# moberweger/deep-prior-pp

Measured on AMD Instinct MI355X. Metric: depth-crops/sec (NYU ResNet50 bs128) 1/2/4/8 GPU; mean 3D joint err (mm), higher is better.
Workload: dtype f32; 1 GPU; NYU posereg_embedding ResNet (type 0, 30-D PCA prior) train step: fused augment + fwd + bwd + ADAM, bs128/GPU fp32, 128x128x1 crops; global_batch=128, parallelism=dp1, augment=True, augment_pipelined=True, bn=local per-GPU batch statistics, launch_mode=native

## Files before the change

deep-prior-pp_amd/csrc/gemm_expand.hip:

```cpp
#include "gemm_args.h"

namespace {

template <int KT, bool BKC, bool IT2, bool ACT, bool RES, bool BNB, bool LZ = false, bool PB = false, bool ST = false>
__global__ __launch_bounds__(DPP_THREADS) DPP_WAVES_PER_EU(1, 2) void gemm_expand_kernel(GemmArgs ga, int rpw) {
    static_assert(!PB || ((KT % 32 == 0 || KT == 16) && !LZ), "bf16 MFMA operands: whole 32-deep steps, or K = 16 with a zero upper half");
    dpp_kernarg_warm<sizeof(GemmArgs)>();
    const dpp_gemm_desc& d = ga.d;
    constexpr int KL = KT / 4, KV = KL / 4;
    constexpr int RT = 2, RI = 16 * RT;
    const int lane = threadIdx.x & 63, l15 = lane & 15, kq = lane >> 4;
    const int NG = d.N >> 6, nblk = d.M / rpw;
    const int gw = blockIdx.x * 4 + (threadIdx.x >> 6);
    if (gw >= NG * nblk) return;
    const int cg = gw % NG, rblk = gw / NG;
    const int n0 = cg * 64 + 4 * l15;
    const int wrow0 = rblk * rpw, iters = rpw / RI;
    const dpp_epilogue& ep = d.epi;
    const int modeA = ACT ? d.actA.mode : 0;
    const bool relu_mask = BNB && ep.bn_relu != 0;
    const bool a16 = ST && !LZ && ga.shA != 0, c16 = ST && (d.store & DPP_ST_C) != 0, x16 = ST && (d.store & DPP_ST_BNX) != 0;
    dpp_stamp(ga.prof, 0);

    float bw[4][KL];
    if (BKC) {
#pragma unroll
        for (int ct = 0; ct < 4; ++ct)
#pragma unroll
            for (int j = 0; j < KV; ++j) {
                const float4 t = *reinterpret_cast<const float4*>(d.B + (size_t)(n0 + ct) * d.ldb + kq * KL + 4 * j);
                bw[ct][4 * j] = t.x; bw[ct][4 * j + 1] = t.y; bw[ct][4 * j + 2] = t.z; bw[ct][4 * j + 3] = t.w;
            }
    } else {
#pragma unroll
        for (int e = 0; e < KL; ++e) {
            const float4 t = *reinterpret_cast<const float4*>(d.B + (size_t)(kq * KL + e) * d.ldb + n0);
            bw[0][e] = t.x; bw[1][e] = t.y; bw[2][e] = t.z; bw[3][e] = t.w;
        }
    }
    constexpr int KS = PB ? (KL + 7) / 8 : 1;
    dpp_bf16x8 bwp[4][KS];
    if (PB) {
#pragma unroll
        for (int ct = 0; ct < 4; ++ct)
#pragma unroll
            for (int ss = 0; ss < KS; ++ss)
#pragma unroll
                for (int q = 0; q < 8; ++q) bwp[ct][ss][q] = (dpp_bf16)(ss * 8 + q < KL ? bw[ct][ss * 8 + q < KL ? ss * 8 + q : 0] : 0.0f);
    }
    struct Regs { float4 a[RT][KV]; float4 a2[RT][LZ ? KV : 1]; float4 res[RT][4]; float4 bx[RT][4]; };
    auto fetch = [&](Regs& g, int it) {
        const int r0 = wrow0 + it * RI;
#pragma unroll
        for (int rt = 0; rt < RT; ++rt) {
            const size_t oa = (size_t)(r0 + rt * 16 + l15) * d.lda + kq * KL;
            if (a16) {
#pragma unroll
                for (int j = 0; j < KV; ++j) g.a[rt][j] = dpp_raw8(d.A + ((oa + 4 * j) >> 1));
            } else {
#pragma unroll
                for (int j = 0; j < KV; ++j) {
                    g.a[rt][j] = *reinterpret_cast<const float4*>(d.A + oa + 4 * j);
                    if (LZ) g.a2[rt][j] = *reinterpret_cast<const float4*>(d.actA.x2 + oa + 4 * j);
                }
            }
        }
#pragma unroll
        for (int rt = 0; rt < RT; ++rt)
#pragma unroll
            for (int r = 0; r < 4; ++r) {
                const size_t o = (size_t)(r0 + rt * 16 + kq * 4 + r) * d.ldc + n0;
                if (RES) g.res[rt][r] = c16 ? dpp_raw8(d.residual + (o >> 1)) : *reinterpret_cast<const float4*>(d.residual + o);
                if (BNB) g.bx[rt][r] = x16 ? dpp_raw8(ep.bn_x + (o >> 1)) : *reinterpret_cast<const float4*>(ep.bn_x + o);
            }
    };
    Regs g0, g1;
    fetch(g0, 0);
    float4 mu[KV], sc[KV], be[KV], ax[LZ ? KV : 1];
#pragma unroll
    for (int j = 0; j < KV; ++j) {
        mu[j] = sc[j] = be[j] = make_float4(0.f, 0.f, 0.f, 0.f);
        if (LZ || (modeA & 2)) {
            mu[j] = *reinterpret_cast<const float4*>(d.actA.mean + kq * KL + 4 * j);
            sc[j] = *reinterpret_cast<const float4*>(d.actA.scale + kq * KL + 4 * j);
            be[j] = *reinterpret_cast<const float4*>(d.actA.beta + kq * KL + 4 * j);
        }
        if (LZ) ax[j] = *reinterpret_cast<const float4*>(d.actA.aux + kq * KL + 4 * j);
    }
    const bool lz_store = LZ && d.actA.out != nullptr && cg == 0;
    float4 cbias = make_float4(0.f, 0.f, 0.f, 0.f), cmean = cbias, cscale = cbias, cbeta = cbias, cistd = cbias;
    if (d.bias) cbias = *reinterpret_cast<const float4*>(d.bias + n0);
    if (BNB) {
        cmean = *reinterpret_cast<const float4*>(ep.bn_mean + n0); cscale = *reinterpret_cast<const float4*>(ep.bn_scale + n0);
        cbeta = *reinterpret_cast<const float4*>(ep.bn_beta + n0); cistd = *reinterpret_cast<const float4*>(ep.bn_inv_std + n0);
    }
    dpp_stamp(ga.prof, 1);

    float sx[4] = {0.f, 0.f, 0.f, 0.f}, sy[4] = {0.f, 0.f, 0.f, 0.f};
    float rmean[4] = {0.f, 0.f, 0.f, 0.f}, rm2[4] = {0.f, 0.f, 0.f, 0.f};
    const bool want_stats = ep.stats != nullptr;
    auto colsum = [&](float (&s)[4]) {
#pragma unroll
        for (int j = 0; j < 4; ++j) { s[j] += __shfl_xor(s[j], 16); s[j] += __shfl_xor(s[j], 32); }
    };

    auto step = [&](Regs& g, int it) {
        const int r0 = wrow0 + it * RI;
        f32x4 acc[RT][4];
#pragma unroll
        for (int rt = 0; rt < RT; ++rt)
#pragma unroll
            for (int ct = 0; ct < 4; ++ct) acc[rt][ct] = (f32x4){0.f, 0.f, 0.f, 0.f};
        dpp_bf16x8 ap[RT][KS];
        if (PB && KL < 8) {
#pragma unroll
            for (int rt = 0; rt < RT; ++rt)
#pragma unroll
                for (int q = 0; q < 8; ++q) ap[rt][0][q] = (dpp_bf16)0.0f;
        }
#pragma unroll
        for (int j = 0; j < KV; ++j) {
            float av[RT][4];
#pragma unroll
            for (int rt = 0; rt < RT; ++rt) {
                float4 v = a16 ? dpp_widen4(g.a[rt][j]) : g.a[rt][j];
                if (LZ) {
                    const float4 x = g.a2[rt][j];
                    v = make_float4(sc[j].x * v.x - ax[j].x * (x.x - mu[j].x) - be[j].x, sc[j].y * v.y - ax[j].y * (x.y - mu[j].y) - be[j].y,
                                    sc[j].z * v.z - ax[j].z * (x.z - mu[j].z) - be[j].z, sc[j].w * v.w - ax[j].w * (x.w - mu[j].w) - be[j].w);
                    if (lz_store) *reinterpret_cast<float4*>(d.actA.out + (size_t)(r0 + rt * 16 + l15) * d.lda + kq * KL + 4 * j) = v;
                }
                if (modeA & 2) {
                    v.x = dpp_fma(v.x - mu[j].x, sc[j].x, be[j].x); v.y = dpp_fma(v.y - mu[j].y, sc[j].y, be[j].y);
                    v.z = dpp_fma(v.z - mu[j].z, sc[j].z, be[j].z); v.w = dpp_fma(v.w - mu[j].w, sc[j].w, be[j].w);
                }
                if (modeA & 1) { v.x = fmaxf(v.x, 0.f); v.y = fmaxf(v.y, 0.f); v.z = fmaxf(v.z, 0.f); v.w = fmaxf(v.w, 0.f); }
                av[rt][0] = v.x; av[rt][1] = v.y; av[rt][2] = v.z; av[rt][3] = v.w;
                if (PB) {
#pragma unroll
                    for (int t = 0; t < 4; ++t) ap[rt][j / 2][(j & 1) * 4 + t] = (dpp_bf16)av[rt][t];
                }
            }
            if (PB) {
                if ((j & 1) || KL < 8) {
#pragma unroll
                    for (int rt = 0; rt < RT; ++rt)
#pragma unroll
                        for (int ct = 0; ct < 4; ++ct)
                            acc[rt][ct] = __builtin_amdgcn_mfma_f32_16x16x32_bf16(ap[rt][j / 2], bwp[ct][j / 2], acc[rt][ct], 0, 0, 0);
                }
            } else {
#pragma unroll
                for (int t = 0; t < 4; ++t)
#pragma unroll
                    for (int rt = 0; rt < RT; ++rt)
#pragma unroll
                        for (int ct = 0; ct < 4; ++ct)
                            acc[rt][ct] = __builtin_amdgcn_mfma_f32_16x16x4f32(av[rt][t], bw[ct][4 * j + t], acc[rt][ct], 0, 0, 0);
            }
        }
        float vals[RT][4][4];
#pragma unroll
        for (int rt = 0; rt < RT; ++rt)
#pragma unroll
            for (int r = 0; r < 4; ++r) {
                float v[4] = {acc[rt][0][r] + cbias.x, acc[rt][1][r] + cbias.y, acc[rt][2][r] + cbias.z, acc[rt][3][r] + cbias.w};
                if (RES) {
                    const float4 rr = c16 ? dpp_widen4(g.res[rt][r]) : g.res[rt][r];
                    v[0] += rr.x; v[1] += rr.y; v[2] += rr.z; v[3] += rr.w;
                }
                if (BNB) {
                    const float4 bxv = x16 ? dpp_widen4(g.bx[rt][r]) : g.bx[rt][r];
                    const float x[4] = {bxv.x, bxv.y, bxv.z, bxv.w};
                    const float cm[4] = {cmean.x, cmean.y, cmean.z, cmean.w}, cs[4] = {cscale.x, cscale.y, cscale.z, cscale.w};
                    const float cb[4] = {cbeta.x, cbeta.y, cbeta.z, cbeta.w}, ci[4] = {cistd.x, cistd.y, cistd.z, cistd.w};
#pragma unroll
                    for (int j = 0; j < 4; ++j) {
                        const float dx = x[j] - cm[j];
                        if (relu_mask && dx * cs[j] + cb[j] < 0.0f) v[j] = 0.0f;
                        if (c16) v[j] = dpp_bf16_round(v[j]);
                        sx[j] += v[j];
                        sy[j] += v[j] * (dx * ci[j]);
                    }
                }
                {
                    const size_t oc = (size_t)(r0 + rt * 16 + kq * 4 + r) * d.ldc + n0;
                    if (c16) dpp_st4(reinterpret_cast<dpp_bf16*>(d.C) + oc, make_float4(v[0], v[1], v[2], v[3]));
                    else *reinterpret_cast<float4*>(d.C + oc) = make_float4(v[0], v[1], v[2], v[3]);
                }
#pragma unroll
                for (int j = 0; j < 4; ++j) vals[rt][r][j] = v[j];
            }
        if (want_stats) {
            float sm[4] = {0.f, 0.f, 0.f, 0.f}, m2[4] = {0.f, 0.f, 0.f, 0.f};
#pragma unroll
            for (int rt = 0; rt < RT; ++rt)
#pragma unroll
                for (int r = 0; r < 4; ++r)
#pragma unroll
                    for (int j = 0; j < 4; ++j) sm[j] += vals[rt][r][j];
            colsum(sm);
#pragma unroll
            for (int j = 0; j < 4; ++j) sm[j] *= 1.0f / (float)RI;
#pragma unroll
            for (int rt = 0; rt < RT; ++rt)
#pragma unroll
                for (int r = 0; r < 4; ++r)
#pragma unroll
                    for (int j = 0; j < 4; ++j) { const float dv = vals[rt][r][j] - sm[j]; m2[j] += dv * dv; }
            colsum(m2);
            if (it == 0) {
#pragma unroll
                for (int j = 0; j < 4; ++j) { rmean[j] = sm[j]; rm2[j] = m2[j]; }
            } else {
                const float na = (float)(it * RI), nb = (float)RI, nn = na + nb;
#pragma unroll
                for (int j = 0; j < 4; ++j) {
                    const float dl = sm[j] - rmean[j];
                    rmean[j] += dl * (nb / nn);
                    rm2[j] += m2[j] + dl * dl * (na * nb / nn);
                }
            }
        }
    };

    if (IT2) {
        for (int it = 0; it < iters; it += 2) {
            if (it + 1 < iters) fetch(g1, it + 1);
            DPP_SCHED_FENCE();
            step(g0, it);
            if (it + 1 < iters) {
                if (it + 2 < iters) fetch(g0, it + 2);
                DPP_SCHED_FENCE();
                step(g1, it + 1);
            }
        }
    } else {
        DPP_SCHED_FENCE();
        step(g0, 0);
    }
    dpp_stamp(ga.prof, 3);
    if (BNB && ep.bn_partial != nullptr) {
        float tx[4] = {sx[0], sx[1], sx[2], sx[3]}, ty[4] = {sy[0], sy[1], sy[2], sy[3]};
        colsum(tx);
        colsum(ty);
        if (kq == 0) {
#pragma unroll
            for (int j = 0; j < 4; ++j) {
                ep.bn_partial[dpp_partial_index(0, n0 + j, rblk, d.N, nblk)] = tx[j];
                ep.bn_partial[dpp_partial_index(1, n0 + j, rblk, d.N, nblk)] = ty[j];
            }
        }
    }
    if (want_stats && kq == 0) {
#pragma unroll
        for (int j = 0; j < 4; ++j) {
            ep.stats[dpp_partial_index(0, n0 + j, rblk, d.N, nblk)] = rmean[j];
            ep.stats[dpp_partial_index(1, n0 + j, rblk, d.N, nblk)] = rm2[j];
        }
    }
    dpp_stamp(ga.prof, 4);
}

}

int dpp_gemm_expand_rows(const dpp_gemm_desc& d, const GemmArgs& ga) {
    if ((d.store & DPP_ST_B) || (d.store && (d.actA.mode & 4))) return 0;
    if (!d.a_kc || d.splitk != 1 || !d.C || !ga.vecA || !ga.vecB || !ga.wide) return 0;
    if (d.K != 16 && d.K != 32 && d.K != 64) return 0;
    if (d.N % 64 || d.M % 32) return 0;
    if (d.mapA.s != 1 || d.mapB.s != 1 || d.mapC.s != 1 || d.actB.mode != 0) return 0;
    if (d.actA.mode != 0 && d.actA.cmod < d.K) return 0;
    if (d.epi.stats && d.epi.bn_x) return 0;
    if (d.b_kc ? (d.epi.bn_x != nullptr || (d.actA.mode & 4)) : (d.actA.mode != 0 && d.actA.mode != 4)) return 0;
    if (d.actA.mode == 4 && d.actA.out && d.lda != d.K) return 0;
    if (d.precision != 0 && (d.precision != 1 || (d.actA.mode & 4))) return 0;
    int rpw = d.bm;
    if (rpw <= 0) rpw = d.M >= 65536 ? 128 : (d.M >= 16384 ? 64 : 32);
    if (rpw % 32 || d.M % rpw) return 0;
    return rpw;
}

namespace {

template <int KT>
int launch_expand(const GemmArgs& ga, int rpw, hipStream_t st) {
    const dpp_gemm_desc& d = ga.d;
    const int waves = (d.M / rpw) * (d.N / 64);
    const dim3 grid(dpp_cdiv(waves, 4));
    const bool it2 = rpw > 32, act = d.actA.mode != 0, res = d.residual != nullptr, bnb = d.epi.bn_x != nullptr, lz = d.actA.mode == 4;
    const bool pb = d.precision == 1;
    const bool stg = d.store != 0;
#define DPP_EXS(K_, I_, A_, R_, B_, L_, P_, S_) DPP_LAUNCH((gemm_expand_kernel<KT, K_, I_, A_, R_, B_, L_, P_, S_>), grid, dim3(DPP_THREADS), 0, st, ga, rpw)
#define DPP_EX(K_, I_, A_, R_, B_, L_, P_) do { if (!(L_) && stg) DPP_EXS(K_, I_, A_, R_, B_, L_, P_, !(L_)); else DPP_EXS(K_, I_, A_, R_, B_, L_, P_, false); } while (0)
#define DPP_EX_P(K_, I_, A_, R_, B_) do { if (pb) { DPP_EX(K_, I_, A_, R_, B_, false, true); break; } \
                                          DPP_EX(K_, I_, A_, R_, B_, false, false); } while (0)
#define DPP_EX_I(K_, A_, R_, B_, L_) do { if (L_) { if (it2) DPP_EX(K_, true, A_, R_, B_, true, false); else DPP_EX(K_, false, A_, R_, B_, true, false); } \
                                          else if (it2) DPP_EX_P(K_, true, A_, R_, B_); else DPP_EX_P(K_, false, A_, R_, B_); } while (0)
#define DPP_EX_R(K_, A_, B_, L_) do { if (res) DPP_EX_I(K_, A_, true, B_, L_); else DPP_EX_I(K_, A_, false, B_, L_); } while (0)
    if (d.b_kc) {
        if (act) DPP_EX_R(true, true, false, false); else DPP_EX_R(true, false, false, false);
    } else if (lz) {
        if (bnb) DPP_EX_R(false, false, true, true); else DPP_EX_R(false, false, false, true);
    } else {
        if (bnb) DPP_EX_R(false, false, true, false); else DPP_EX_R(false, false, false, false);
    }
#undef DPP_EX_P
#undef DPP_EXS
#undef DPP_EX_R
#undef DPP_EX_I
#undef DPP_EX
    return dpp_launch_status();
}

}

int dpp_gemm_expand_launch(const GemmArgs& ga, int rpw, hipStream_t st) {
    const dpp_gemm_desc& d = ga.d;
    return d.K == 64 ? launch_expand<64>(ga, rpw, st) : (d.K == 32 ? launch_expand<32>(ga, rpw, st) : launch_expand<16>(ga, rpw, st));
}
```

deep-prior-pp_amd/csrc/stem.hip:

```cpp
#include "dpp_common.h"

namespace {

constexpr int KS = 5, PAD = 2, NTAP = 25, KPAD = 28;
constexpr int TC = 16;
constexpr int LX = TC + 2 * PAD;
constexpr int LXP = LX + 1;

template <int CN>
__global__ __launch_bounds__(DPP_THREADS) void stem_fwd_kernel(const float* __restrict__ X, int N, int H, int W, const float* __restrict__ Wk,
                                                               const float* __restrict__ bias, int Co, float* __restrict__ Y,
                                                               uint8_t* __restrict__ arg, int tiles_x, int tiles_y,
                                                               float* __restrict__ stats, int y16) {
    dpp_kernarg_warm<128>();
    __shared__ float xs[LX * LXP];
    __shared__ float Ws[KPAD * CN * 16];
    const int tid = threadIdx.x, wave = tid >> 6, lane = tid & 63, l15 = lane & 15, kq = lane >> 4;
    const int bx = blockIdx.x % tiles_x, by = (blockIdx.x / tiles_x) % tiles_y, n = blockIdx.x / (tiles_x * tiles_y);
    const int cy0 = by * TC, cx0 = bx * TC;
    const int Hp = H >> 1, Wp = W >> 1;
    const float* img = X + (size_t)n * H * W;
    for (int s = tid; s < LX * LX; s += DPP_THREADS) {
        int hy = s / LX, hx = s - hy * LX;
        int y = cy0 + hy - PAD, x = cx0 + hx - PAD;
        xs[hy * LXP + hx] = (y >= 0 && y < H && x >= 0 && x < W) ? img[(size_t)y * W + x] : 0.0f;
    }
    for (int s = tid; s < KPAD * CN * 16; s += DPP_THREADS) {
        int k = s / (CN * 16), o = s - k * (CN * 16);
        Ws[s] = (k < NTAP && o < Co) ? Wk[(size_t)o * NTAP + k] : 0.0f;
    }
    __syncthreads();

    float bf[7][CN];
#pragma unroll
    for (int t = 0; t < 7; ++t)
#pragma unroll
        for (int ct = 0; ct < CN; ++ct) bf[t][ct] = Ws[(4 * t + kq) * (CN * 16) + ct * 16 + l15];
    int koff[7];
    bool kval[7];
#pragma unroll
    for (int t = 0; t < 7; ++t) {
        int k = 4 * t + kq;
        kval[t] = k < NTAP;
        int kk = kval[t] ? k : 0;
        koff[t] = (kk / KS) * LXP + (kk % KS);
    }

    float vals[4][CN];
#pragma unroll
    for (int i = 0; i < 4; ++i)
#pragma unroll
        for (int j = 0; j < CN; ++j) vals[i][j] = 0.0f;
#pragma unroll
    for (int rt = 0; rt < 4; ++rt) {
        const int ply = 2 * wave + (rt >> 1);
        const int qa = l15 >> 2, pa = l15 & 3;
        const int ay = 2 * ply + (pa >> 1), ax = 2 * (((rt & 1) << 2) + qa) + (pa & 1);
        const int abase = ay * LXP + ax;
        f32x4 acc[CN];
#pragma unroll
        for (int ct = 0; ct < CN; ++ct) acc[ct] = (f32x4){0.f, 0.f, 0.f, 0.f};
#pragma unroll
        for (int t = 0; t < 7; ++t) {
            float av = kval[t] ? xs[abase + koff[t]] : 0.0f;
#pragma unroll
            for (int ct = 0; ct < CN; ++ct) acc[ct] = __builtin_amdgcn_mfma_f32_16x16x4f32(av, bf[t][ct], acc[ct], 0, 0, 0);
        }
        const int py = (cy0 >> 1) + ply, px = (cx0 >> 1) + ((rt & 1) << 2) + kq;
        if (py < Hp && px < Wp) {
            size_t o = (((size_t)n * Hp + py) * Wp + px) * Co;
#pragma unroll
            for (int ct = 0; ct < CN; ++ct) {
                int col = ct * 16 + l15;
                if (col < Co) {
                    float best = fmaxf(fmaxf(acc[ct][0], acc[ct][1]), fmaxf(acc[ct][2], acc[ct][3]));
                    int ties = 0;
#pragma unroll
                    for (int r = 0; r < 4; ++r) ties |= (acc[ct][r] == best) ? (1 << r) : 0;
                    if (y16) reinterpret_cast<dpp_bf16*>(Y)[o + col] = (dpp_bf16)(best + bias[col]);
                    else Y[o + col] = best + bias[col];
                    vals[rt][ct] = best + bias[col];
                    if (arg) arg[o + col] = (uint8_t)ties;
                }
            }
        }
    }
    if (stats != nullptr) {
        float sm[CN], m2[CN];
#pragma unroll
        for (int ct = 0; ct < CN; ++ct) sm[ct] = vals[0][ct] + vals[1][ct] + vals[2][ct] + vals[3][ct];
        dpp_tile_colsum<CN, 4, 1, CN * 16>(sm, xs, wave, 0, l15, kq);
#pragma unroll
        for (int ct = 0; ct < CN; ++ct) {
            sm[ct] *= (1.0f / 64.0f);
            float t = 0.0f;
#pragma unroll
            for (int rt = 0; rt < 4; ++rt) { float dv = vals[rt][ct] - sm[ct]; t += dv * dv; }
            m2[ct] = t;
        }
        dpp_tile_colsum<CN, 4, 1, CN * 16>(m2, xs, wave, 0, l15, kq);
        if (kq == 0 && wave == 0) {
#pragma unroll
            for (int ct = 0; ct < CN; ++ct) {
                int col = ct * 16 + l15;
                if (col < Co) {
                    stats[dpp_partial_index(0, col, blockIdx.x, Co, gridDim.x)] = sm[ct];
                    stats[dpp_partial_index(1, col, blockIdx.x, Co, gridDim.x)] = m2[ct];
                }
            }
        }
    }
}

constexpr int LXW = LX + 2;
constexpr int GM_A = 64 * 32 + 16;

__global__ __launch_bounds__(DPP_THREADS) void stem_wgrad_kernel(const float* __restrict__ X, int N, int H, int W, const float* __restrict__ dY,
                                                                 const uint8_t* __restrict__ arg, int Co, float* __restrict__ partial,
                                                                 int tiles_x, int tiles_y, int tiles_per_block, int total_tiles) {
    dpp_kernarg_warm<128>();
    __shared__ __attribute__((aligned(16))) float gm[4 * GM_A];
    __shared__ float xs[LX * LXW];
    const int tid = threadIdx.x, wave = tid >> 6, lane = tid & 63, l15 = lane & 15, kq = lane >> 4;
    const int Hp = H >> 1, Wp = W >> 1;
    const bool vec = (Co & 3) == 0 && (reinterpret_cast<uintptr_t>(dY) & 15) == 0 && (reinterpret_cast<uintptr_t>(arg) & 3) == 0;
    int offB[2];
    bool okB[2];
#pragma unroll
    for (int ct = 0; ct < 2; ++ct) {
        const int tap = ct * 16 + l15;
        okB[ct] = tap < NTAP;
        const int tt = okB[ct] ? tap : 0;
        offB[ct] = ((kq >> 1) + tt / KS) * LXW + (kq & 1) + tt % KS;
    }
    float4 rg[2];
    unsigned rt_[2];
    float rh[2];
    auto load_tile = [&](int tile) {
        const int bx = tile % tiles_x, by = (tile / tiles_x) % tiles_y, n = tile / (tiles_x * tiles_y);
        const int cy0 = by * TC, cx0 = bx * TC;
#pragma unroll
        for (int i = 0; i < 2; ++i) {
            const int item = tid + i * DPP_THREADS, p = item >> 3, oq = item & 7;
            const int py = (cy0 >> 1) + (p >> 3), px = (cx0 >> 1) + (p & 7);
            float4 g = make_float4(0.f, 0.f, 0.f, 0.f);
            unsigned t = 0;
            if (py < Hp && px < Wp && oq * 4 < Co) {
                const size_t idx = (((size_t)n * Hp + py) * Wp + px) * Co + oq * 4;
                if (vec) {
                    g = *reinterpret_cast<const float4*>(dY + idx);
                    t = *reinterpret_cast<const unsigned*>(arg + idx);
                } else {
                    float gv[4] = {0.f, 0.f, 0.f, 0.f};
                    for (int j = 0; j < 4; ++j)
                        if (oq * 4 + j < Co) { gv[j] = dY[idx + j]; t |= (unsigned)arg[idx + j] << (8 * j); }
                    g = make_float4(gv[0], gv[1], gv[2], gv[3]);
                }
            }
            rg[i] = g;
            rt_[i] = t;
        }
        const float* img = X + (size_t)n * H * W;
#pragma unroll
        for (int i = 0; i < 2; ++i) {
            const int s2 = tid + i * DPP_THREADS;
            float v = 0.0f;
            if (s2 < LX * LX) {
                const int hy = s2 / LX, hx = s2 - hy * LX;
                const int y = cy0 + hy - PAD, x = cx0 + hx - PAD;
                if (y >= 0 && y < H && x >= 0 && x < W) v = img[(size_t)y * W + x];
            }
            rh[i] = v;
        }
    };
    auto commit_tile = [&]() {
#pragma unroll
        for (int i = 0; i < 2; ++i) {
            const int item = tid + i * DPP_THREADS, p = item >> 3, oq = item & 7;
            const float4 g = rg[i];
            const unsigned t = rt_[i];
#pragma unroll
            for (int a = 0; a < 4; ++a) {
                float4 m;
                m.x = ((t >> a) & 1u) ? g.x : 0.0f;
                m.y = ((t >> (8 + a)) & 1u) ? g.y : 0.0f;
                m.z = ((t >> (16 + a)) & 1u) ? g.z : 0.0f;
                m.w = ((t >> (24 + a)) & 1u) ? g.w : 0.0f;
                *reinterpret_cast<float4*>(&gm[a * GM_A + p * 32 + oq * 4]) = m;
            }
        }
#pragma unroll
        for (int i = 0; i < 2; ++i) {
            const int s2 = tid + i * DPP_THREADS;
            if (s2 < LX * LX) xs[(s2 / LX) * LXW + s2 % LX] = rh[i];
        }
    };
    f32x4 acc[2][2];
#pragma unroll
    for (int i = 0; i < 2; ++i)
#pragma unroll
        for (int j = 0; j < 2; ++j) acc[i][j] = (f32x4){0.f, 0.f, 0.f, 0.f};
    const int tile0 = blockIdx.x * tiles_per_block;
    int ntiles = total_tiles - tile0;
    if (ntiles > tiles_per_block) ntiles = tiles_per_block;
    if (ntiles > 0) load_tile(tile0);
    for (int ti = 0; ti < ntiles; ++ti) {
        commit_tile();
        __syncthreads();
        if (ti + 1 < ntiles) load_tile(tile0 + ti + 1);
#pragma unroll
        for (int sidx = 0; sidx < 16; ++sidx) {
            const int p = wave * 16 + sidx;
            const int base = (2 * (p >> 3)) * LXW + 2 * (p & 7);
            const float a0 = gm[kq * GM_A + p * 32 + l15], a1 = gm[kq * GM_A + p * 32 + 16 + l15];
            const float b0 = okB[0] ? xs[base + offB[0]] : 0.0f;
            const float b1 = okB[1] ? xs[base + offB[1]] : 0.0f;
            acc[0][0] = __builtin_amdgcn_mfma_f32_16x16x4f32(a0, b0, acc[0][0], 0, 0, 0);
            acc[0][1] = __builtin_amdgcn_mfma_f32_16x16x4f32(a0, b1, acc[0][1], 0, 0, 0);
            acc[1][0] = __builtin_amdgcn_mfma_f32_16x16x4f32(a1, b0, acc[1][0], 0, 0, 0);
            acc[1][1] = __builtin_amdgcn_mfma_f32_16x16x4f32(a1, b1, acc[1][1], 0, 0, 0);
        }
        __syncthreads();
    }
    float* red = gm;
#pragma unroll
    for (int rt = 0; rt < 2; ++rt)
#pragma unroll
        for (int ct = 0; ct < 2; ++ct)
#pragma unroll
            for (int r = 0; r < 4; ++r) red[wave * 1024 + (rt * 16 + kq * 4 + r) * 32 + ct * 16 + l15] = acc[rt][ct][r];
    __syncthreads();
    for (int s2 = tid; s2 < Co * NTAP; s2 += DPP_THREADS) {
        const int oo = s2 / NTAP, k = s2 - oo * NTAP;
        const int at = oo * 32 + k;
        partial[(size_t)blockIdx.x * Co * NTAP + s2] = ((red[at] + red[1024 + at]) + red[2048 + at]) + red[3072 + at];
    }
}

}

extern "C" int dpp_stem_fwd(const float* X, int N, int H, int W, const float* Wk, const float* bias, int Co, float* Y, uint8_t* argmax,
                            float* stats, int store,
                            dpp_stream_t stream) {
    if (!X || !Wk || !bias || !Y || N < 1 || H < 2 || W < 2 || (H & 1) || (W & 1) || Co < 1 || Co > 32 || (store & ~DPP_ST_C)) return DPP_E_BADARG;
    const int y16 = (store & DPP_ST_C) ? 1 : 0;
    if (stats && ((H % TC) || (W % TC))) return DPP_E_BADARG;
    int tiles_x = dpp_cdiv(W, TC), tiles_y = dpp_cdiv(H, TC);
    dim3 grid(tiles_x * tiles_y * N);
    hipStream_t st = static_cast<hipStream_t>(stream);
    if (Co <= 16)
        DPP_LAUNCH((stem_fwd_kernel<1>), grid, dim3(DPP_THREADS), 0, st, X, N, H, W, Wk, bias, Co, Y, argmax, tiles_x, tiles_y, stats, y16);
    else
        DPP_LAUNCH((stem_fwd_kernel<2>), grid, dim3(DPP_THREADS), 0, st, X, N, H, W, Wk, bias, Co, Y, argmax, tiles_x, tiles_y, stats, y16);
    return dpp_launch_status();
}

extern "C" int dpp_stem_wgrad_blocks(int N, int H, int W, int tiles_per_block) {
    int total = dpp_cdiv(W, TC) * dpp_cdiv(H, TC) * N;
    return dpp_cdiv(total, tiles_per_block > 0 ? tiles_per_block : 1);
}

extern "C" int dpp_stem_wgrad(const float* X, int N, int H, int W, const float* dY, const uint8_t* argmax, int Co, float* partial,
                              int tiles_per_block, dpp_stream_t stream) {
    if (!X || !dY || !argmax || !partial || N < 1 || (H & 1) || (W & 1) || Co < 1 || Co > 32 || tiles_per_block < 1)
        return DPP_E_BADARG;
    int tiles_x = dpp_cdiv(W, TC), tiles_y = dpp_cdiv(H, TC);
    int total = tiles_x * tiles_y * N;
    DPP_LAUNCH(stem_wgrad_kernel, dim3(dpp_cdiv(total, tiles_per_block)), dim3(DPP_THREADS), 0, static_cast<hipStream_t>(stream), X, N,
                       H, W, dY, argmax, Co, partial, tiles_x, tiles_y, tiles_per_block, total);
    return dpp_launch_status();
}
```

Measured before the change: 37990 depth-crops/sec.

## Stage K-contiguous B tile through swizzled LDS in expand GEMM

For K-contiguous B (b_kc) with K at least 64, all four waves of a block now share one 64-column group. They cooperatively load that B tile with coalesced float4 reads into an XOR-swizzled shared-memory buffer, and each wave then reads its fragment from LDS. Before, every wave did its own strided per-lane global loads of B. The grid is remapped so a block covers one column group and four row blocks. Waves past the last row block stay alive only to help with staging. This adds a __syncthreads and LDS usage per block, and it changes the block-to-tile mapping, which can affect occupancy and L2 locality.

```diff
diff --git a/deep-prior-pp_amd/csrc/gemm_expand.hip b/deep-prior-pp_amd/csrc/gemm_expand.hip
--- a/deep-prior-pp_amd/csrc/gemm_expand.hip
+++ b/deep-prior-pp_amd/csrc/gemm_expand.hip
@@ -1,9 +1,10 @@
+#include <stdlib.h>
 #include "gemm_args.h"
 
 namespace {
 
 template <int KT, bool BKC, bool IT2, bool ACT, bool RES, bool BNB, bool LZ = false, bool PB = false, bool ST = false>
-__global__ __launch_bounds__(DPP_THREADS) DPP_WAVES_PER_EU(1, 2) void gemm_expand_kernel(GemmArgs ga, int rpw) {
+__global__ __launch_bounds__(DPP_THREADS) DPP_WAVES_PER_EU(1, 2) void gemm_expand_kernel(GemmArgs ga, int rpw, int ldsb) {
     static_assert(!PB || ((KT % 32 == 0 || KT == 16) && !LZ), "bf16 MFMA operands: whole 32-deep steps, or K = 16 with a zero upper half");
     dpp_kernarg_warm<sizeof(GemmArgs)>();
     const dpp_gemm_desc& d = ga.d;
@@ -11,9 +12,12 @@
     constexpr int RT = 2, RI = 16 * RT;
     const int lane = threadIdx.x & 63, l15 = lane & 15, kq = lane >> 4;
     const int NG = d.N >> 6, nblk = d.M / rpw;
+    const bool stage_b = BKC && ldsb != 0;
     const int gw = blockIdx.x * 4 + (threadIdx.x >> 6);
-    if (gw >= NG * nblk) return;
-    const int cg = gw % NG, rblk = gw / NG;
+    if (!stage_b && gw >= NG * nblk) return;
+    const int cg = stage_b ? (int)blockIdx.x % NG : gw % NG;
+    const int rblk = stage_b ? ((int)blockIdx.x / NG) * 4 + (int)(threadIdx.x >> 6) : gw / NG;
+    const bool live = rblk < nblk;
     const int n0 = cg * 64 + 4 * l15;
     const int wrow0 = rblk * rpw, iters = rpw / RI;
     const dpp_epilogue& ep = d.epi;
@@ -22,8 +26,19 @@
     const bool a16 = ST && !LZ && ga.shA != 0, c16 = ST && (d.store & DPP_ST_C) != 0, x16 = ST && (d.store & DPP_ST_BNX) != 0;
     dpp_stamp(ga.prof, 0);
 
+    __shared__ f32x4 bstage[BKC ? 16 * KT : 1];
+    constexpr int SW = 4 / KV;
+    f32x4 stg[KV];
+    if (stage_b) {
+#pragma unroll
+        for (int i = 0; i < KV; ++i) {
+            const int f = i * DPP_THREADS + (int)threadIdx.x, n = f / (KT / 4), q = f % (KT / 4);
+            stg[i] = *reinterpret_cast<const f32x4*>(d.B + (size_t)(cg * 64 + n) * d.ldb + 4 * q);
+        }
+    }
     float bw[4][KL];
-    if (BKC) {
+    if (stage_b) {
+    } else if (BKC) {
 #pragma unroll
         for (int ct = 0; ct < 4; ++ct)
 #pragma unroll
@@ -39,15 +54,6 @@
         }
     }
     constexpr int KS = PB ? (KL + 7) / 8 : 1;
-    dpp_bf16x8 bwp[4][KS];
-    if (PB) {
-#pragma unroll
-        for (int ct = 0; ct < 4; ++ct)
-#pragma unroll
-            for (int ss = 0; ss < KS; ++ss)
-#pragma unroll
-                for (int q = 0; q < 8; ++q) bwp[ct][ss][q] = (dpp_bf16)(ss * 8 + q < KL ? bw[ct][ss * 8 + q < KL ? ss * 8 + q : 0] : 0.0f);
-    }
     struct Regs { float4 a[RT][KV]; float4 a2[RT][LZ ? KV : 1]; float4 res[RT][4]; float4 bx[RT][4]; };
     auto fetch = [&](Regs& g, int it) {
         const int r0 = wrow0 + it * RI;
@@ -75,7 +81,7 @@
             }
     };
     Regs g0, g1;
-    fetch(g0, 0);
+    if (live) fetch(g0, 0);
     float4 mu[KV], sc[KV], be[KV], ax[LZ ? KV : 1];
 #pragma unroll
     for (int j = 0; j < KV; ++j) {
@@ -93,6 +99,34 @@
     if (BNB) {
         cmean = *reinterpret_cast<const float4*>(ep.bn_mean + n0); cscale = *reinterpret_cast<const float4*>(ep.bn_scale + n0);
         cbeta = *reinterpret_cast<const float4*>(ep.bn_beta + n0); cistd = *reinterpret_cast<const float4*>(ep.bn_inv_std + n0);
+    }
+    if (stage_b) {
+        DPP_SCHED_FENCE();
+#pragma unroll
+        for (int i = 0; i < KV; ++i) {
+            const int f = i * DPP_THREADS + (int)threadIdx.x, n = f / (KT / 4), q = f % (KT / 4);
+            const int v = (n & 3) * KV + q % KV;
+            bstage[v * 64 + (q / KV) * 16 + (((n >> 2) & 15) ^ (v * SW))] = stg[i];
+        }
+        __syncthreads();
+        if (!live) return;
+#pragma unroll
+        for (int ct = 0; ct < 4; ++ct)
+#pragma unroll
+            for (int j = 0; j < KV; ++j) {
+                const int v = ct * KV + j;
+                const f32x4 t = bstage[v * 64 + kq * 16 + (l15 ^ (v * SW))];
+                bw[ct][4 * j] = t[0]; bw[ct][4 * j + 1] = t[1]; bw[ct][4 * j + 2] = t[2]; bw[ct][4 * j + 3] = t[3];
+            }
+    }
+    dpp_bf16x8 bwp[4][KS];
+    if (PB) {
+#pragma unroll
+        for (int ct = 0; ct < 4; ++ct)
+#pragma unroll
+            for (int ss = 0; ss < KS; ++ss)
+#pragma unroll
+                for (int q = 0; q < 8; ++q) bwp[ct][ss][q] = (dpp_bf16)(ss * 8 + q < KL ? bw[ct][ss * 8 + q < KL ? ss * 8 + q : 0] : 0.0f);
     }
     dpp_stamp(ga.prof, 1);
 
@@ -287,11 +321,13 @@
 int launch_expand(const GemmArgs& ga, int rpw, hipStream_t st) {
     const dpp_gemm_desc& d = ga.d;
     const int waves = (d.M / rpw) * (d.N / 64);
-    const dim3 grid(dpp_cdiv(waves, 4));
+    static const int lds_b = []() { const char* e = getenv("DPP_EXPAND_LDS_B"); return e && e[0] ? atoi(e) : 1; }();
+    const int ldsb = (d.b_kc && lds_b > 0 && KT >= (lds_b == 1 ? 64 : (lds_b == 2 ? 32 : 16))) ? 1 : 0;
+    const dim3 grid(ldsb ? (d.N / 64) * dpp_cdiv(d.M / rpw, 4) : dpp_cdiv(waves, 4));
     const bool it2 = rpw > 32, act = d.actA.mode != 0, res = d.residual != nullptr, bnb = d.epi.bn_x != nullptr, lz = d.actA.mode == 4;
     const bool pb = d.precision == 1;
     const bool stg = d.store != 0;
-#define DPP_EXS(K_, I_, A_, R_, B_, L_, P_, S_) DPP_LAUNCH((gemm_expand_kernel<KT, K_, I_, A_, R_, B_, L_, P_, S_>), grid, dim3(DPP_THREADS), 0, st, ga, rpw)
+#define DPP_EXS(K_, I_, A_, R_, B_, L_, P_, S_) DPP_LAUNCH((gemm_expand_kernel<KT, K_, I_, A_, R_, B_, L_, P_, S_>), grid, dim3(DPP_THREADS), 0, st, ga, rpw, ldsb)
 #define DPP_EX(K_, I_, A_, R_, B_, L_, P_) do { if (!(L_) && stg) DPP_EXS(K_, I_, A_, R_, B_, L_, P_, !(L_)); else DPP_EXS(K_, I_, A_, R_, B_, L_, P_, false); } while (0)
 #define DPP_EX_P(K_, I_, A_, R_, B_) do { if (pb) { DPP_EX(K_, I_, A_, R_, B_, false, true); break; } \
                                           DPP_EX(K_, I_, A_, R_, B_, false, false); } while (0)
```

Result: no change. 37960 depth-crops/sec (-0.1%).

## Add persistent double-buffered stem forward kernel walking tiles with prefetch

Applied to the files above, without the earlier changes.

Adds a persistent stem conv+pool forward kernel launched with a capped grid (default 1024 blocks) that loops over tiles. It loads the weights into LDS and registers once per block and double-buffers the input halo tile, prefetching the next tile's pixels into registers while the current tile's MFMA work runs. This targets repeated per-block weight staging and exposed global-load latency in the one-tile-per-block kernel. The cost is less parallelism per tile, an extra LDS buffer, and an environment-variable knob. It only applies to Co of 16 or 32 with aligned outputs.

```diff
diff --git a/deep-prior-pp_amd/csrc/stem.hip b/deep-prior-pp_amd/csrc/stem.hip
--- a/deep-prior-pp_amd/csrc/stem.hip
+++ b/deep-prior-pp_amd/csrc/stem.hip
@@ -1,3 +1,4 @@
+#include <stdlib.h>
 #include "dpp_common.h"
 
 namespace {
@@ -112,6 +113,187 @@
     }
 }
 
+template <int CN>
+__global__ __launch_bounds__(DPP_THREADS) void stem_walk_kernel(const float* __restrict__ X, int H, int W, const float* __restrict__ Wk,
+                                                                const float* __restrict__ bias, float* __restrict__ Y,
+                                                                uint8_t* __restrict__ arg, int tiles_x, int tiles_y, int ntiles,
+                                                                float* __restrict__ stats, int y16) {
+    dpp_kernarg_warm<96>();
+    constexpr int Co = CN * 16;
+    constexpr int XSZ = LX * LXP;
+    __shared__ float xs[2 * XSZ];
+    __shared__ float Ws[KPAD * Co];
+    __shared__ float red[4 * Co];
+    const int tid = threadIdx.x, wave = tid >> 6, lane = tid & 63, l15 = lane & 15, kq = lane >> 4;
+    const int Hp = H >> 1, Wp = W >> 1;
+
+    int hy[2], hx[2], hoff[2];
+    bool hon[2];
+#pragma unroll
+    for (int u = 0; u < 2; ++u) {
+        const int s = tid + u * DPP_THREADS;
+        hon[u] = s < LX * LX;
+        hy[u] = s / LX;
+        hx[u] = s - hy[u] * LX;
+        hoff[u] = hon[u] ? hy[u] * LXP + hx[u] : 0;
+    }
+    const int dx = (int)gridDim.x % tiles_x, dy = ((int)gridDim.x / tiles_x) % tiles_y, dn = (int)gridDim.x / (tiles_x * tiles_y);
+    int fbx = (int)blockIdx.x % tiles_x, fby = ((int)blockIdx.x / tiles_x) % tiles_y, fn = (int)blockIdx.x / (tiles_x * tiles_y);
+    float hr[2];
+    unsigned hin = 0;
+    auto fetch = [&](bool more) {
+        const int cy0 = fby * TC, cx0 = fbx * TC;
+        const float* img = X + (more ? (size_t)fn * H * W : (size_t)0);
+        hin = 0;
+#pragma unroll
+        for (int u = 0; u < 2; ++u) {
+            const int y = cy0 + hy[u] - PAD, x = cx0 + hx[u] - PAD;
+            const bool in = more && hon[u] && y >= 0 && y < H && x >= 0 && x < W;
+            hin |= in ? (1u << u) : 0u;
+            hr[u] = img[in ? y * W + x : 0];
+        }
+    };
+    auto commit = [&](float* xc) {
+#pragma unroll
+        for (int u = 0; u < 2; ++u)
+            if (hon[u]) xc[hoff[u]] = ((hin >> u) & 1u) ? hr[u] : 0.0f;
+    };
+    auto advance = [&]() {
+        fbx += dx;
+        if (fbx >= tiles_x) { fbx -= tiles_x; ++fby; }
+        fby += dy;
+        if (fby >= tiles_y) { fby -= tiles_y; ++fn; }
+        fn += dn;
+    };
+    int tile = blockIdx.x;
+    fetch(tile < ntiles);
+    for (int s = tid; s < KPAD * Co; s += DPP_THREADS) {
+        int k = s / Co, o = s - k * Co;
+        Ws[s] = k < NTAP ? Wk[(size_t)o * NTAP + k] : 0.0f;
+    }
+    commit(xs);
+    __syncthreads();
+
+    float bf[7][CN];
+#pragma unroll
+    for (int t = 0; t < 7; ++t)
+#pragma unroll
+        for (int ct = 0; ct < CN; ++ct) bf[t][ct] = Ws[(4 * t + kq) * Co + CN * l15 + ct];
+    int koff[7];
+    bool kval[7];
+#pragma unroll
+    for (int t = 0; t < 7; ++t) {
+        int k = 4 * t + kq;
+        kval[t] = k < NTAP;
+        int kk = kval[t] ? k : 0;
+        koff[t] = (kk / KS) * LXP + (kk % KS);
+    }
+    float bv[CN];
+#pragma unroll
+    for (int ct = 0; ct < CN; ++ct) bv[ct] = bias[CN * l15 + ct];
+#ifndef DPP_HIP_EMU
+#pragma unroll
+    for (int ct = 0; ct < CN; ++ct) asm volatile("" ::"v"(bv[ct]));
+#endif
+    int abase[4];
+#pragma unroll
+    for (int rt = 0; rt < 4; ++rt) {
+        const int ply = 2 * wave + (rt >> 1);
+        const int qa = l15 >> 2, pa = l15 & 3;
+        const int ay = 2 * ply + (pa >> 1), ax = 2 * (((rt & 1) << 2) + qa) + (pa & 1);
+        abase[rt] = ay * LXP + ax;
+    }
+
+    int cur = 0;
+    for (; tile < ntiles; tile += gridDim.x) {
+        const float* const xc = xs + cur * XSZ;
+        const int n = fn, cy0 = fby * TC, cx0 = fbx * TC;
+        __syncthreads();
+        advance();
+        fetch(tile + (int)gridDim.x < ntiles);
+
+        float vals[4][CN];
+        unsigned tbs[4];
+#pragma unroll
+        for (int rt = 0; rt < 4; ++rt) {
+            f32x4 acc[CN];
+#pragma unroll
+            for (int ct = 0; ct < CN; ++ct) acc[ct] = (f32x4){0.f, 0.f, 0.f, 0.f};
+#pragma unroll
+            for (int t = 0; t < 7; ++t) {
+                float av = kval[t] ? xc[abase[rt] + koff[t]] : 0.0f;
+#pragma unroll
+                for (int ct = 0; ct < CN; ++ct) acc[ct] = __builtin_amdgcn_mfma_f32_16x16x4f32(av, bf[t][ct], acc[ct], 0, 0, 0);
+            }
+            unsigned tb = 0;
+#pragma unroll
+            for (int ct = 0; ct < CN; ++ct) {
+                float best = fmaxf(fmaxf(acc[ct][0], acc[ct][1]), fmaxf(acc[ct][2], acc[ct][3]));
+                unsigned ties = 0;
+#pragma unroll
+                for (int r = 0; r < 4; ++r) ties |= (acc[ct][r] == best) ? (1u << r) : 0u;
+                vals[rt][ct] = best + bv[ct];
+                tb |= ties << (8 * ct);
+            }
+            tbs[rt] = tb;
+        }
+        commit(xs + (cur ^ 1) * XSZ);
+#pragma unroll
+        for (int rt = 0; rt < 4; ++rt) {
+            const int py = (cy0 >> 1) + 2 * wave + (rt >> 1), px = (cx0 >> 1) + ((rt & 1) << 2) + kq;
+            const size_t o = (((size_t)n * Hp + py) * Wp + px) * Co + CN * l15;
+            unsigned tb = tbs[rt];
+            if (y16) {
+                dpp_bf16* y = reinterpret_cast<dpp_bf16*>(Y) + o;
+                if constexpr (CN == 2) {
+                    const dpp_bf16 lo = (dpp_bf16)vals[rt][0], hi = (dpp_bf16)vals[rt][1];
+                    unsigned short ul, uh;
+                    __builtin_memcpy(&ul, &lo, 2);
+                    __builtin_memcpy(&uh, &hi, 2);
+                    *reinterpret_cast<unsigned*>(y) = (unsigned)ul | ((unsigned)uh << 16);
+                } else y[0] = (dpp_bf16)vals[rt][0];
+            } else {
+                if constexpr (CN == 2) *reinterpret_cast<float2*>(Y + o) = make_float2(vals[rt][0], vals[rt][1]);
+                else Y[o] = vals[rt][0];
+            }
+            if (arg != nullptr) {
+                if constexpr (CN == 2) {
+                    tb |= (unsigned)__shfl_xor((int)tb, 1) << 16;
+                    if ((l15 & 1) == 0) *reinterpret_cast<unsigned*>(arg + o) = tb;
+                } else {
+                    tb <<= 8 * (l15 & 3);
+                    tb |= (unsigned)__shfl_xor((int)tb, 1);
+                    tb |= (unsigned)__shfl_xor((int)tb, 2);
+                    if ((l15 & 3) == 0) *reinterpret_cast<unsigned*>(arg + o) = tb;
+                }
+            }
+        }
+        if (stats != nullptr) {
+            float sm[CN], m2[CN];
+#pragma unroll
+            for (int ct = 0; ct < CN; ++ct) sm[ct] = vals[0][ct] + vals[1][ct] + vals[2][ct] + vals[3][ct];
+            dpp_tile_colsum<CN, 4, 1, Co>(sm, red, wave, 0, l15, kq);
+#pragma unroll
+            for (int ct = 0; ct < CN; ++ct) {
+                sm[ct] *= (1.0f / 64.0f);
+                float t = 0.0f;
+#pragma unroll
+                for (int rt = 0; rt < 4; ++rt) { float dv = vals[rt][ct] - sm[ct]; t += dv * dv; }
+                m2[ct] = t;
+            }
+            dpp_tile_colsum<CN, 4, 1, Co>(m2, red, wave, 0, l15, kq);
+            if (kq == 0 && wave == 0) {
+#pragma unroll
+                for (int ct = 0; ct < CN; ++ct) {
+                    stats[dpp_partial_index(0, CN * l15 + ct, tile, Co, ntiles)] = sm[ct];
+                    stats[dpp_partial_index(1, CN * l15 + ct, tile, Co, ntiles)] = m2[ct];
+                }
+            }
+        }
+        cur ^= 1;
+    }
+}
+
 constexpr int LXW = LX + 2;
 constexpr int GM_A = 64 * 32 + 16;
 
@@ -248,6 +430,18 @@
     int tiles_x = dpp_cdiv(W, TC), tiles_y = dpp_cdiv(H, TC);
     dim3 grid(tiles_x * tiles_y * N);
     hipStream_t st = static_cast<hipStream_t>(stream);
+    const char* we = getenv("DPP_STEM_WALK");
+    const int walk = we ? atoi(we) : 1024;
+    const bool aligned = (reinterpret_cast<uintptr_t>(Y) & 7) == 0 && (!argmax || (reinterpret_cast<uintptr_t>(argmax) & 3) == 0);
+    if (walk > 0 && H % TC == 0 && W % TC == 0 && (Co == 16 || Co == 32) && aligned) {
+        const int ntiles = tiles_x * tiles_y * N;
+        const dim3 gw(walk < ntiles ? walk : ntiles);
+        if (Co == 16)
+            DPP_LAUNCH((stem_walk_kernel<1>), gw, dim3(DPP_THREADS), 0, st, X, H, W, Wk, bias, Y, argmax, tiles_x, tiles_y, ntiles, stats, y16);
+        else
+            DPP_LAUNCH((stem_walk_kernel<2>), gw, dim3(DPP_THREADS), 0, st, X, H, W, Wk, bias, Y, argmax, tiles_x, tiles_y, ntiles, stats, y16);
+        return dpp_launch_status();
+    }
     if (Co <= 16)
         DPP_LAUNCH((stem_fwd_kernel<1>), grid, dim3(DPP_THREADS), 0, st, X, N, H, W, Wk, bias, Co, Y, argmax, tiles_x, tiles_y, stats, y16);
     else
```

New measurement: 37810 depth-crops/sec before, 38010 depth-crops/sec after, median of 6. About the same (+0.5%).

## Add persistent tile-walking stem forward kernel with prefetched input and MFMA conv

Applied to the files above, without the earlier changes.

Adds a persistent stem forward kernel that walks tiles with a fixed grid (default 1280 workgroups). It prefetches the next tile's input into registers while computing the current one, keeps weights in registers across tiles, and stages outputs and argmax ties through shared memory for vectorized stores. It is specialized on train/eval and the bf16 output mode, and writes per-tile BN partial stats. The aim is to cut per-block launch and setup overhead and hide global load latency. The cost is more shared memory, a register budget set by waves-per-EU, and a new stats indexing layout that must match its consumers.

```diff
diff --git a/deep-prior-pp_amd/csrc/stem.hip b/deep-prior-pp_amd/csrc/stem.hip
--- a/deep-prior-pp_amd/csrc/stem.hip
+++ b/deep-prior-pp_amd/csrc/stem.hip
@@ -112,6 +112,196 @@
     }
 }
 
+constexpr int XP = 44;
+constexpr int XSZ = LX * XP;
+
+template <int CN, bool TRAIN, bool Y16>
+__global__ __launch_bounds__(DPP_THREADS) DPP_WAVES_PER_EU(5, 8) void stem_fwd_walk_kernel(const float* __restrict__ X, int H, int W, const float* __restrict__ Wk,
+                                                                    const float* __restrict__ bias, int Co, float* __restrict__ Y,
+                                                                    uint8_t* __restrict__ arg, int tiles_x, int tiles_y, int ntiles,
+                                                                    float* __restrict__ stats) {
+    dpp_kernarg_warm<128>();
+    constexpr int NC = CN * 16;
+    constexpr int YP = CN == 2 ? 48 : 16;
+    constexpr int LQ = CN == 2 ? 3 : 2;
+    __shared__ __attribute__((aligned(16))) float xs[XSZ];
+    __shared__ __attribute__((aligned(16))) float Ys[64 * YP];
+    __shared__ __attribute__((aligned(16))) uint8_t ts[TRAIN ? 64 * NC + DPP_THREADS : 16];
+    __shared__ float red[TRAIN ? 2 * 4 * NC : 1];
+    const int tid = threadIdx.x, wave = tid >> 6, lane = tid & 63, l15 = lane & 15, kq = lane >> 4;
+    const int G = gridDim.x;
+    int tile = blockIdx.x;
+    if (tile >= ntiles) return;
+    const int Hp = H >> 1, Wp = W >> 1;
+
+    float bf[7][CN], bv[CN];
+#pragma unroll
+    for (int ct = 0; ct < CN; ++ct) {
+        const int col = ct * 16 + l15;
+        const bool cok = col < Co;
+#pragma unroll
+        for (int t = 0; t < 7; ++t) {
+            const int k = 4 * t + kq;
+            const bool ok = cok && k < NTAP;
+            const float w = Wk[ok ? col * NTAP + k : 0];
+            bf[t][ct] = ok ? w : 0.0f;
+        }
+        const float b = bias[cok ? col : 0];
+        bv[ct] = cok ? b : 0.0f;
+    }
+    const int qa = l15 >> 2, pa = l15 & 3;
+    const int abase = (4 * wave + (pa >> 1)) * XP + 2 * qa + (pa & 1) + 2;
+    const bool kval6 = 24 + kq < NTAP;
+    int aoff[7];
+#pragma unroll
+    for (int t = 0; t < 7; ++t) {
+        const int k = 4 * t + kq, kk = k < NTAP ? k : 0;
+        aoff[t] = abase + (kk / KS) * XP + (kk % KS);
+    }
+    const int p0 = 16 * wave + kq;
+    const int ybase = p0 * YP + l15;
+    const bool lastok = (CN - 1) * 16 + l15 < Co;
+    int tbase[4], tlast[4];
+#pragma unroll
+    for (int rt = 0; rt < 4; ++rt) {
+        tbase[rt] = (p0 + (rt >> 1) * 8 + (rt & 1) * 4) * Co + l15;
+        tlast[rt] = lastok ? tbase[rt] + (CN - 1) * 16 : 64 * NC + tid;
+    }
+    const int srow = tid >> 3, sc = tid & 7;
+    const bool sact = tid < LX * 8 && sc < 6;
+    unsigned yoff[CN];
+    bool yok[CN];
+#pragma unroll
+    for (int i = 0; i < CN; ++i) {
+        const int item = tid + i * DPP_THREADS, p = item >> LQ, q = item & ((1 << LQ) - 1);
+        yok[i] = q * 4 < Co;
+        yoff[i] = (unsigned)(((p >> 3) * Wp + (p & 7)) * Co + q * 4);
+    }
+    const int trow = tid >> 4, tpc = tid & 15;
+    const bool tok = tid < 128 && tpc * 2 < Co;
+    const unsigned toff = (unsigned)(trow * Wp * Co + tpc * 16);
+    const unsigned HW = (unsigned)(H * W);
+    const int sy = srow - PAD, sx = sc * 4 - 4;
+    int bx = tile % tiles_x, by = (tile / tiles_x) % tiles_y, n = tile / (tiles_x * tiles_y);
+    const int gx = G % tiles_x, gy = (G / tiles_x) % tiles_y, gn = G / (tiles_x * tiles_y);
+
+    float4 rh = make_float4(0.f, 0.f, 0.f, 0.f);
+    bool rok = false;
+    auto request = [&](int rbx, int rby, int rn) {
+        const int y = rby * TC + sy, x = rbx * TC + sx;
+        rok = sact & ((unsigned)y < (unsigned)H) & ((unsigned)x < (unsigned)W);
+        const unsigned off = rok ? (unsigned)(y * W + x) : 0u;
+        rh = *reinterpret_cast<const float4*>(X + (unsigned)rn * HW + off);
+    };
+    auto commit = [&]() {
+        if (sact) *reinterpret_cast<float4*>(&xs[srow * XP + sc * 4]) = rok ? rh : make_float4(0.f, 0.f, 0.f, 0.f);
+    };
+    request(bx, by, n);
+    commit();
+    __syncthreads();
+
+    for (;; tile += G) {
+        const unsigned obase = (unsigned)(((n * Hp + by * (TC / 2)) * Wp + bx * (TC / 2)) * Co);
+        bx += gx;
+        if (bx >= tiles_x) { bx -= tiles_x; ++by; }
+        by += gy;
+        if (by >= tiles_y) { by -= tiles_y; ++n; }
+        n += gn;
+        const bool more = tile + G < ntiles;
+        if (more) request(bx, by, n);
+        DPP_SCHED_FENCE();
+        float vals[4][CN];
+#pragma unroll
+        for (int rt = 0; rt < 4; ++rt) {
+            const int roff = (rt >> 1) * 2 * XP + (rt & 1) * 8;
+            f32x4 acc[CN];
+#pragma unroll
+            for (int ct = 0; ct < CN; ++ct) acc[ct] = (f32x4){0.f, 0.f, 0.f, 0.f};
+#pragma unroll
+            for (int t = 0; t < 7; ++t) {
+                float av = xs[aoff[t] + roff];
+                if (t == 6) av = kval6 ? av : 0.0f;
+#pragma unroll
+                for (int ct = 0; ct < CN; ++ct) acc[ct] = __builtin_amdgcn_mfma_f32_16x16x4f32(av, bf[t][ct], acc[ct], 0, 0, 0);
+            }
+            const int po = ((rt >> 1) * 8 + (rt & 1) * 4) * YP;
+#pragma unroll
+            for (int ct = 0; ct < CN; ++ct) {
+                float best = fmaxf(fmaxf(acc[ct][0], acc[ct][1]), fmaxf(acc[ct][2], acc[ct][3]));
+                vals[rt][ct] = best + bv[ct];
+                Ys[ybase + po + ct * 16] = vals[rt][ct];
+                if (TRAIN) {
+                    int ties = 0;
+#pragma unroll
+                    for (int r = 0; r < 4; ++r) ties |= (acc[ct][r] == best) ? (1 << r) : 0;
+                    ts[ct == CN - 1 ? tlast[rt] : tbase[rt] + ct * 16] = (uint8_t)ties;
+                }
+            }
+        }
+        float sm[CN], m2[CN];
+        if (TRAIN) {
+#pragma unroll
+            for (int ct = 0; ct < CN; ++ct) sm[ct] = vals[0][ct] + vals[1][ct] + vals[2][ct] + vals[3][ct];
+            dpp_tile_colsum<CN, 1, 1, NC>(sm, red, 0, 0, l15, kq);
+            if (kq == 0) {
+#pragma unroll
+                for (int ct = 0; ct < CN; ++ct) red[wave * NC + ct * 16 + l15] = sm[ct];
+            }
+        }
+        __syncthreads();
+        if (more) commit();
+#pragma unroll
+        for (int i = 0; i < CN; ++i) {
+            const int item = tid + i * DPP_THREADS, p = item >> LQ, q = item & ((1 << LQ) - 1);
+            if (yok[i]) {
+                const float4 v = *reinterpret_cast<const float4*>(&Ys[p * YP + q * 4]);
+                if (Y16) dpp_st4(reinterpret_cast<dpp_bf16*>(Y) + obase + yoff[i], v);
+                else dpp_st4(Y + obase + yoff[i], v);
+            }
+        }
+        if (TRAIN) {
+            if (tok) *reinterpret_cast<uint4*>(arg + obase + toff) = *reinterpret_cast<const uint4*>(&ts[trow * 8 * Co + tpc * 16]);
+#pragma unroll
+            for (int ct = 0; ct < CN; ++ct) {
+                float t = 0.0f;
+#pragma unroll
+                for (int w = 0; w < 4; ++w) t += red[w * NC + ct * 16 + l15];
+                sm[ct] = t;
+            }
+#pragma unroll
+            for (int ct = 0; ct < CN; ++ct) {
+                sm[ct] *= (1.0f / 64.0f);
+                float t = 0.0f;
+#pragma unroll
+                for (int rt = 0; rt < 4; ++rt) { float dv = vals[rt][ct] - sm[ct]; t += dv * dv; }
+                m2[ct] = t;
+            }
+            dpp_tile_colsum<CN, 1, 1, NC>(m2, red, 0, 0, l15, kq);
+            if (kq == 0) {
+#pragma unroll
+                for (int ct = 0; ct < CN; ++ct) red[4 * NC + wave * NC + ct * 16 + l15] = m2[ct];
+            }
+        }
+        __syncthreads();
+        if (TRAIN) {
+            if (kq == 0 && wave == 0) {
+#pragma unroll
+                for (int ct = 0; ct < CN; ++ct) {
+                    const int col = ct * 16 + l15;
+                    float t = 0.0f;
+#pragma unroll
+                    for (int w = 0; w < 4; ++w) t += red[4 * NC + w * NC + ct * 16 + l15];
+                    if (col < Co) {
+                        stats[(unsigned)(col * ntiles + tile)] = sm[ct];
+                        stats[(unsigned)((Co + col) * ntiles + tile)] = t;
+                    }
+                }
+            }
+        }
+        if (!more) break;
+    }
+}
+
 constexpr int LXW = LX + 2;
 constexpr int GM_A = 64 * 32 + 16;
 
@@ -248,6 +438,24 @@
     int tiles_x = dpp_cdiv(W, TC), tiles_y = dpp_cdiv(H, TC);
     dim3 grid(tiles_x * tiles_y * N);
     hipStream_t st = static_cast<hipStream_t>(stream);
+    const char* fe = getenv("DPP_STEM_FWD");
+    const char* we = getenv("DPP_STEM_FWD_WGS");
+    const int wgs = (we && atoi(we) > 0) ? atoi(we) : 1280;
+    auto al16 = [](const void* p) { return (reinterpret_cast<uintptr_t>(p) & 15) == 0; };
+    const bool train = argmax != nullptr && stats != nullptr, eval = argmax == nullptr && stats == nullptr;
+    if (!(fe && fe[0] == '0') && H % TC == 0 && W % TC == 0 && Co % 4 == 0 && (train || eval) && al16(X) && al16(Y) && al16(argmax) &&
+        (long)N * H * W < (1L << 31) && (long)N * (H / 2) * (W / 2) * Co < (1L << 31)) {
+        const int ntiles = tiles_x * tiles_y * N;
+        const dim3 gw(ntiles < wgs ? ntiles : wgs);
+#define DPP_STEMW(CN_, T_, Y_) DPP_LAUNCH((stem_fwd_walk_kernel<CN_, T_, Y_>), gw, dim3(DPP_THREADS), 0, st, X, H, W, Wk, bias, Co, Y, argmax, tiles_x, tiles_y, ntiles, stats)
+#define DPP_STEMW_Y(CN_, T_) do { if (y16) DPP_STEMW(CN_, T_, true); else DPP_STEMW(CN_, T_, false); } while (0)
+#define DPP_STEMW_T(CN_) do { if (train) DPP_STEMW_Y(CN_, true); else DPP_STEMW_Y(CN_, false); } while (0)
+        if (Co <= 16) DPP_STEMW_T(1); else DPP_STEMW_T(2);
+#undef DPP_STEMW_T
+#undef DPP_STEMW_Y
+#undef DPP_STEMW
+        return dpp_launch_status();
+    }
     if (Co <= 16)
         DPP_LAUNCH((stem_fwd_kernel<1>), grid, dim3(DPP_THREADS), 0, st, X, N, H, W, Wk, bias, Co, Y, argmax, tiles_x, tiles_y, stats, y16);
     else
```

After: 37750 depth-crops/sec before, 37950 depth-crops/sec after (median of 6 runs). Within noise of the previous version (+0.5%).
